# SerCharles/CN-RMA

Measured on AMD Instinct MI355X. Metric: scenes/sec fwd (40-view->192^3 voxel): dense unprojection + RMA + voxelise + FCAF3D + decode, higher is better.
Workload: dtype f32 (sparse conv f16x3: 22-bit operands, fp32 accumulate; value_f32_conv = exact fp32); 1 GPU; NS: 40 views x 256 ch x 480x640 fp32 maps (channels_last) -> grid 192x192x192, N=300, max_points=500000, FCAF3D MinkResNet34 + head, 1 HIP graph per scene, 3 in flight; M_rows=72216505, M_selected=500000, M_unique=496819

## Files before the change

### cn-rma_amd/csrc/rma.hip

```cpp
#include "common.h"

#include <stdlib.h>

namespace {

struct MarchParams {
  int V, H, W, X, Y, Z, N;
  float vs, ox, oy, oz, t_one, thr;
};

struct Ray {
  float ox, oy, oz, dx, dy, dz;
};

__device__ __forceinline__ Ray make_ray(const float* __restrict__ Pi, float u, float v) {
  float far_[3], o[3];
#pragma unroll
  for (int r = 0; r < 3; ++r) {
    float acc = Pi[r * 4 + 0] * u;
    acc = fmaf(Pi[r * 4 + 1], v, acc);
    acc = fmaf(Pi[r * 4 + 2], 1.0f, acc);
    acc = fmaf(Pi[r * 4 + 3], 1.0f, acc);
    far_[r] = acc;
    o[r] = Pi[r * 4 + 3];
// ... 722 lines not shown
  } else {
    if (tsdf == nullptr) return CNRMA_EINVAL;
    hipLaunchKernelGGL(neus_count_kernel, dim3((unsigned)ceil_div(R, 256)), dim3(256), 0, st, p, proj_inv, tsdf, count, wsum,
                       reinterpret_cast<int2*>(kept), cap, overflow);
  }
  CNRMA_LAUNCH_CHECK();
  return 0;
}

extern "C" int cnrma_rma_neus_march_f32(const float* proj_inv, const float* tsdf, const float* sig_table, int V, int H,
                                        int W, int X, int Y, int Z, float voxel_size, float ox, float oy, float oz,
                                        int n_steps, float t_one, float thr, int32_t* count, double* wsum, void* kept,
                                        int cap, int32_t* overflow, const void* skip_table, void* stream) {
  if (bad_dims(V, H, W, X, Y, Z, n_steps) || kept == nullptr || cap <= 0 || overflow == nullptr) return CNRMA_EINVAL;
  if (tsdf == nullptr && sig_table == nullptr) return CNRMA_EINVAL;
  MarchParams p = make_params(V, H, W, X, Y, Z, voxel_size, ox, oy, oz, n_steps, t_one, thr);
  return launch_march(p, proj_inv, tsdf, sig_table, count, wsum, kept, cap, overflow, nullptr, nullptr, 0, as_stream(stream),
                      sig_table ? reinterpret_cast<const uint8_t*>(skip_table) : nullptr);
}

extern "C" int cnrma_nchw_to_nhwc_march_f32(const float* feat_nchw, float* feat_nhwc, int C, const float* proj_inv,
                                            const float* tsdf, const float* sig_table, int V, int H, int W, int X, int Y,
                                            int Z, float voxel_size, float ox, float oy, float oz, int n_steps, float t_one,
                                            float thr, int32_t* count, double* wsum, void* kept, int cap, int32_t* overflow,
                                            const void* skip_table, void* stream) {
  if (bad_dims(V, H, W, X, Y, Z, n_steps) || kept == nullptr || cap <= 0 || overflow == nullptr || C <= 0 ||
      feat_nchw == nullptr || feat_nhwc == nullptr)
    return CNRMA_EINVAL;
  if (tsdf == nullptr && sig_table == nullptr) return CNRMA_EINVAL;
  MarchParams p = make_params(V, H, W, X, Y, Z, voxel_size, ox, oy, oz, n_steps, t_one, thr);
  return launch_march(p, proj_inv, tsdf, sig_table, count, wsum, kept, cap, overflow, feat_nchw, feat_nhwc, C, as_stream(stream),
                      sig_table ? reinterpret_cast<const uint8_t*>(skip_table) : nullptr);
}

template <int ELEM = 0, typename FT = float>
static int neus_emit_rows_any(const float* proj_inv, const FT* feat_nhwc, const FT* const* feat_ref, int V, int C, int H, int W,
                                            int n_steps, float t_one, const int32_t* row_offset, int64_t n_out,
                                            const int32_t* n_out_dev, const void* kept, int cap,
                                            const int32_t* sel_index, int64_t sel_cap, void* records,
                                            const float* w_div, float addx, float addy, float addz, float* out_xyz,
                                            int xyz_stride, float* out_w, int w_stride, float* out_feat,
                                            int feat_stride, int32_t* out_sample, void* stream) {
  if (V <= 0 || C <= 0 || H <= 0 || W <= 0 || n_out <= 0 || (kept != nullptr && cap <= 0) || records == nullptr ||
      (kept == nullptr && row_offset != nullptr) || (feat_nhwc == nullptr && feat_ref == nullptr && out_feat != nullptr))
    return CNRMA_EINVAL;
  MarchParams p = make_params(V, H, W, 1, 1, 1, 1.0f, 0.f, 0.f, 0.f, n_steps, t_one, 0.0f);
  EmitDst d{out_xyz, xyz_stride, out_w, w_stride, out_feat, feat_stride, out_sample, nullptr, w_div, addx, addy, addz};
  const int64_t R = (int64_t)V * H * W;
  hipStream_t st = as_stream(stream);
  int4* rec = reinterpret_cast<int4*>(records);
  if (kept != nullptr)
    hipLaunchKernelGGL(neus_scatter_records_kernel, dim3((unsigned)ceil_div(R, 256)), dim3(256), 0, st, R, row_offset,
                       reinterpret_cast<const int2*>(kept), cap, sel_index, sel_cap, n_out, rec);
  if (C % 256 == 0) {
    hipLaunchKernelGGL((neus_emit_rows_kernel<64, ELEM, FT>), dim3((unsigned)ceil_div(n_out * 64, 256)), dim3(256), 0, st, p, C,
                       proj_inv, feat_nhwc, feat_ref, n_out, n_out_dev, rec, d);
  } else if (C % 32 == 0) {
    hipLaunchKernelGGL((neus_emit_rows_kernel<8, ELEM, FT>), dim3((unsigned)ceil_div(n_out * 8, 256)), dim3(256), 0, st, p, C,
                       proj_inv, feat_nhwc, feat_ref, n_out, n_out_dev, rec, d);
  } else {
    hipLaunchKernelGGL((neus_emit_rows_kernel<2, ELEM, FT>), dim3((unsigned)ceil_div(n_out * 2, 256)), dim3(256), 0, st, p, C,
                       proj_inv, feat_nhwc, feat_ref, n_out, n_out_dev, rec, d);
  }
  CNRMA_LAUNCH_CHECK();
  return 0;
}

extern "C" int cnrma_rma_neus_emit_rows_f32(const float* proj_inv, const float* feat_nhwc, int V, int C, int H, int W,
                                            int n_steps, float t_one, const int32_t* row_offset, int64_t n_out,
                                            const int32_t* n_out_dev, const void* kept, int cap,
                                            const int32_t* sel_index, int64_t sel_cap, void* records,
                                            const float* w_div, float addx, float addy, float addz, float* out_xyz,
                                            int xyz_stride, float* out_w, int w_stride, float* out_feat,
                                            int feat_stride, int32_t* out_sample, void* stream) {
  return neus_emit_rows_any<0, float>(proj_inv, feat_nhwc, nullptr, V, C, H, W, n_steps, t_one, row_offset, n_out, n_out_dev, kept, cap,
                            sel_index, sel_cap, records, w_div, addx, addy, addz, out_xyz, xyz_stride, out_w, w_stride, out_feat,
                            feat_stride, out_sample, stream);
}

extern "C" int cnrma_rma_neus_emit_rows_ref_f32(const float* proj_inv, const float* const* feat_nhwc_ref, int V, int C, int H,
                                                int W, int n_steps, float t_one, const int32_t* row_offset, int64_t n_out,
                                                const int32_t* n_out_dev, const void* kept, int cap,
                                                const int32_t* sel_index, int64_t sel_cap, void* records,
                                                const float* w_div, float addx, float addy, float addz, float* out_xyz,
                                                int xyz_stride, float* out_w, int w_stride, float* out_feat,
                                                int feat_stride, int32_t* out_sample, void* stream) {
  if (feat_nhwc_ref == nullptr) return CNRMA_EINVAL;
  return neus_emit_rows_any<0, float>(proj_inv, nullptr, feat_nhwc_ref, V, C, H, W, n_steps, t_one, row_offset, n_out, n_out_dev, kept, cap,
                            sel_index, sel_cap, records, w_div, addx, addy, addz, out_xyz, xyz_stride, out_w, w_stride, out_feat,
                            feat_stride, out_sample, stream);
}

extern "C" int cnrma_rma_neus_emit_rows_h16(const float* proj_inv, const void* feat_nhwc, const void* const* feat_nhwc_ref, int elem,
                                            int V, int C, int H, int W, int n_steps, float t_one, const int32_t* row_offset,
                                            int64_t n_out, const int32_t* n_out_dev, const void* kept, int cap,
                                            const int32_t* sel_index, int64_t sel_cap, void* records, const float* w_div,
                                            float addx, float addy, float addz, float* out_xyz, int xyz_stride, float* out_w,
                                            int w_stride, float* out_feat, int feat_stride, int32_t* out_sample, void* stream) {
  if (!elem16_known(elem) || (feat_nhwc == nullptr) == (feat_nhwc_ref == nullptr) || C % 8 != 0 ||
      (reinterpret_cast<uintptr_t>(feat_nhwc) & 15) != 0)
    return CNRMA_EINVAL;
  const uint16_t* f = static_cast<const uint16_t*>(feat_nhwc);
  const uint16_t* const* fr = reinterpret_cast<const uint16_t* const*>(feat_nhwc_ref);
  if (elem == CNRMA_ELEM_F16)
    return neus_emit_rows_any<CNRMA_ELEM_F16, uint16_t>(proj_inv, f, fr, V, C, H, W, n_steps, t_one, row_offset, n_out, n_out_dev, kept,
                                                        cap, sel_index, sel_cap, records, w_div, addx, addy, addz, out_xyz, xyz_stride,
                                                        out_w, w_stride, out_feat, feat_stride, out_sample, stream);
// ... 139 lines not shown
```

### cn-rma_amd/csrc/sparse.hip

```cpp
#include <cstdio>
#include <type_traits>
#include "common.h"
#include "f16x3.h"

#include <hipcub/hipcub.hpp>

namespace {

struct UniqueWs {
  int32_t* slot;
  int32_t* idx;
  uint8_t* flag;
  void* scan;
  uint64_t* key_a; uint64_t* key_b;
  int32_t* val_a; int32_t* val_b;
  void* sort_tmp; size_t sort_tmp_bytes;
  int32_t* range_err;
};

size_t sort_temp_bytes(int64_t n) {
  size_t bytes = 0;
  hipError_t e = hipcub::DeviceRadixSort::SortPairs(nullptr, bytes, (const uint64_t*)nullptr, (uint64_t*)nullptr,
                                                    (const int32_t*)nullptr, (int32_t*)nullptr, (int)n, 0, 64, nullptr);
  if (e != hipSuccess || bytes == 0) bytes = (size_t)n * 16 + (1u << 20);
// ... 2121 lines not shown
#endif

__global__ __launch_bounds__(256) void convtr_coords_kernel(const int32_t* __restrict__ in_coords, int64_t n_cap,
                                                            const int32_t* __restrict__ n_dev, int half,
                                                            int32_t* __restrict__ out_coords) {
  const int64_t n = live_rows(n_cap, n_dev);
  const int64_t t = (int64_t)blockIdx.x * blockDim.x + threadIdx.x;
  if (t >= n * 8) return;
  const int m = (int)(t & 7);
  const int64_t i = t >> 3;
  int4 c = reinterpret_cast<const int4*>(in_coords)[i];
  c.y += ((m >> 2) & 1) * half;
  c.z += ((m >> 1) & 1) * half;
  c.w += (m & 1) * half;
  reinterpret_cast<int4*>(out_coords)[t] = c;
}

__global__ __launch_bounds__(256) void maxpool_kernel(const float* __restrict__ in, int C, const int32_t* __restrict__ nbr,
                                                      int K, float* __restrict__ out, int64_t no_cap,
                                                      const int32_t* __restrict__ no_dev) {
  const int64_t n = live_rows(no_cap, no_dev);
  const int64_t t = (int64_t)blockIdx.x * blockDim.x + threadIdx.x;
  if ((C & 3) == 0) {
    const int c4 = C >> 2;
    if (t >= n * c4) return;
    const int64_t o = t / c4;
    const int c = (int)(t - o * c4);
    float4 m = make_float4(-__builtin_inff(), -__builtin_inff(), -__builtin_inff(), -__builtin_inff());
    bool any = false;
    for (int k = 0; k < K; ++k) {
      const int32_t s = nbr[o * K + k];
      if (s >= 0) {
        const float4 v = reinterpret_cast<const float4*>(in)[(int64_t)s * c4 + c];
        m.x = fmaxf(m.x, v.x); m.y = fmaxf(m.y, v.y); m.z = fmaxf(m.z, v.z); m.w = fmaxf(m.w, v.w);
        any = true;
      }
    }
    reinterpret_cast<float4*>(out)[t] = any ? m : make_float4(0.f, 0.f, 0.f, 0.f);
    return;
  }
  if (t >= n * C) return;
  const int64_t o = t / C;
  const int c = (int)(t - o * C);
  float m = -__builtin_inff();
  bool any = false;
  for (int k = 0; k < K; ++k) {
    int32_t s = nbr[o * K + k];
    if (s >= 0) { m = fmaxf(m, in[(int64_t)s * C + c]); any = true; }
  }
  out[t] = any ? m : 0.0f;
}

struct StatsTerm {
  const float* __restrict__ in;
  __device__ __forceinline__ void operator()(int64_t i, double& a, double& b) const {
    const double v = (double)in[i];
    a = v;
    b = v * v;
  }
};

__device__ __forceinline__ void mask_grad(float& g, float yv, int act) {
  if (!(yv > 0.0f)) g = act == 2 ? g * (yv + 1.0f) : 0.0f;
}

struct GradTerm {
  const float* __restrict__ dy; const float* __restrict__ x; const float* __restrict__ y; int act;
  __device__ __forceinline__ void operator()(int64_t i, double& a, double& b) const {
    float gf = dy[i];
    if (y != nullptr) mask_grad(gf, y[i], act);
    const double g = (double)gf;
    a = g;
    b = g * (double)x[i];
  }
};

template <typename Term>
__global__ __launch_bounds__(256) void colsum_partial_kernel(Term term, int64_t n_cap, const int32_t* __restrict__ n_dev,
                                                             const int32_t* __restrict__ row0_dev, int C,
                                                             double* __restrict__ part) {
  const int64_t n = live_rows(n_cap, n_dev);
  const int64_t i0 = row0_dev != nullptr ? (int64_t)__builtin_nontemporal_load(row0_dev) * C : 0;
  const int c = threadIdx.x % C;
  const int groups = blockDim.x / C;
  const int gi = threadIdx.x / C;
  double s = 0.0, q = 0.0;
  if (gi < groups) {
    for (int64_t r = (int64_t)blockIdx.x * groups + gi; r < n; r += (int64_t)gridDim.x * groups) {
      double a, b;
      term(i0 + r * C + c, a, b);
      s += a;
      q += b;
    }
  }
  __shared__ double sm[2 * 256];
  sm[threadIdx.x] = s;
  sm[256 + threadIdx.x] = q;
  __syncthreads();
  if (threadIdx.x < C) {
    double ts = 0.0, tq = 0.0;
    for (int g = 0; g < groups; ++g) { ts += sm[g * C + threadIdx.x]; tq += sm[256 + g * C + threadIdx.x]; }
    part[(int64_t)blockIdx.x * 2 * C + threadIdx.x] = ts;
    part[(int64_t)blockIdx.x * 2 * C + C + threadIdx.x] = tq;
  }
}

__device__ __forceinline__ void colsum_channel(const double* __restrict__ part, int nblk, int C, int c, double& s_out, double& q_out) {
  __shared__ double ss[256], qq[256];
  double s = 0.0, q = 0.0;
  for (int b = threadIdx.x; b < nblk; b += 256) { s += part[(int64_t)b * 2 * C + c]; q += part[(int64_t)b * 2 * C + C + c]; }
  ss[threadIdx.x] = s; qq[threadIdx.x] = q;
  __syncthreads();
  for (int d = 128; d > 0; d >>= 1) {
    if ((int)threadIdx.x < d) { ss[threadIdx.x] += ss[threadIdx.x + d]; qq[threadIdx.x] += qq[threadIdx.x + d]; }
    __syncthreads();
  }
  if (threadIdx.x == 0) { s_out = ss[0]; q_out = qq[0]; }
}

__global__ __launch_bounds__(256) void colstats_final_kernel(const double* __restrict__ part, int nblk, int C, int64_t n_cap,
                                                             const int32_t* __restrict__ n_dev, double* __restrict__ stats,
                                                             float momentum, float* __restrict__ running_mean,
                                                             float* __restrict__ running_var, int64_t* __restrict__ batches) {
  const int c = blockIdx.x;
  double s = 0.0, q = 0.0;
  colsum_channel(part, nblk, C, c, s, q);
  if (threadIdx.x == 0) {
    const double nn = (double)live_rows(n_cap, n_dev);
    const double mean = s / nn;
    double var = q / nn - mean * mean;
    if (var < 0.0) var = 0.0;
    stats[c] = mean;
    stats[C + c] = var;
    if (running_mean != nullptr) running_mean[c] = (1.0f - momentum) * running_mean[c] + momentum * (float)mean;
    if (running_var != nullptr) running_var[c] = (1.0f - momentum) * running_var[c] + momentum * (float)(var * (nn / (nn - 1.0)));
    if (batches != nullptr && c == 0) *batches += 1;
  }
}

__global__ __launch_bounds__(256) void bn_backward_final_kernel(const double* __restrict__ part, int nblk, int C, int64_t n,
                                                                const double* __restrict__ stats, float eps,
                                                                float* __restrict__ dweight, float* __restrict__ dbias,
                                                                double* __restrict__ sums) {
  const int c = blockIdx.x;
  double s = 0.0, q = 0.0;
  colsum_channel(part, nblk, C, c, s, q);
  if (threadIdx.x == 0) {
    const double mean = stats[c], inv = 1.0 / sqrt(stats[C + c] + (double)eps);
    const double dg = (q - mean * s) * inv;
    if (dweight) dweight[c] = (float)dg;
// ... 15 lines not shown
  float v = (x - k.mean) * k.inv;
  if (weight) v = v * weight[c];
  if (bias) v = v + bias[c];
  return v;
}

__device__ __forceinline__ float norm_backward(float g, float x, NormCoef k, const float* weight,
                                               const double* sums, int C, int c) {
  const double* sums2 = sums + C;
  const float xhat = (x - k.mean) * k.inv;
  const float gain = weight ? weight[c] : 1.0f;
  return gain * k.inv * (g - (float)sums[c] - xhat * (float)sums2[c]);
}

__global__ __launch_bounds__(256) void instnorm_apply_kernel(const float* __restrict__ in, int64_t n_cap,
                                                             const int32_t* __restrict__ n_dev,
                                                             const int32_t* __restrict__ row0_dev, int C,
                                                             const double* __restrict__ stats,
                                                             const float* __restrict__ weight,
                                                             const float* __restrict__ bias, float eps, int relu,
                                                             float* __restrict__ out) {
  const int64_t n = live_rows(n_cap, n_dev);
  if (row0_dev != nullptr) {
    const int64_t r0 = (int64_t)__builtin_nontemporal_load(row0_dev) * C;
    in += r0;
    out += r0;
  }
  for (int64_t t = (int64_t)blockIdx.x * blockDim.x + threadIdx.x; t < n * C; t += (int64_t)gridDim.x * blockDim.x) {
    const int c = (int)(t % C);
    const float v = norm_forward(in[t], norm_coef(stats, C, c, eps), weight, bias, c);
    out[t] = relu ? fmaxf(v, 0.0f) : v;
  }
}

__global__ __launch_bounds__(256) void instnorm_maxpool_kernel(const float* __restrict__ in, int C,
                                                               const double* __restrict__ stats,
                                                               const float* __restrict__ weight,
                                                               const float* __restrict__ bias, float eps, int relu,
                                                               const int32_t* __restrict__ nbr, int K, float* __restrict__ out,
                                                               int64_t no_cap, const int32_t* __restrict__ no_dev,
                                                               float* __restrict__ out_amax) {
  const int64_t n = live_rows(no_cap, no_dev);
  const int64_t t = (int64_t)blockIdx.x * blockDim.x + threadIdx.x;
  const int c4 = C >> 2;
  float mx = 0.0f;
  if (t < n * c4) {
    const int64_t o = t / c4;
    const int c = (int)(t - o * c4) * 4;
    NormCoef kc[4];
#pragma unroll
    for (int j = 0; j < 4; ++j) kc[j] = norm_coef(stats, C, c + j, eps);
    float m[4] = {-__builtin_inff(), -__builtin_inff(), -__builtin_inff(), -__builtin_inff()};
    bool any = false;
    for (int k = 0; k < K; ++k) {
      const int32_t s_ = nbr[o * K + k];
      if (s_ >= 0) {
        const float4 q = *reinterpret_cast<const float4*>(in + (int64_t)s_ * C + c);
        const float x[4] = {q.x, q.y, q.z, q.w};
#pragma unroll
        for (int j = 0; j < 4; ++j) {
          float v = norm_forward(x[j], kc[j], weight, bias, c + j);
          if (relu) v = fmaxf(v, 0.0f);
          m[j] = fmaxf(m[j], v);
        }
        any = true;
      }
    }
    float4 r = any ? make_float4(m[0], m[1], m[2], m[3]) : make_float4(0.f, 0.f, 0.f, 0.f);
    *reinterpret_cast<float4*>(out + o * C + c) = r;
    mx = fmaxf(fmaxf(fabsf(r.x), fabsf(r.y)), fmaxf(fabsf(r.z), fabsf(r.w)));
  }
  if (out_amax != nullptr) {
    __shared__ float sh4[4];
    block_amax_publish(out_amax, mx, sh4);
  }
}

__global__ __launch_bounds__(256) void bn_apply_kernel(const float* __restrict__ in, int64_t n, int C, const double* __restrict__ stats,
                                                       const float* __restrict__ weight, const float* __restrict__ bias, float eps,
                                                       const float* __restrict__ residual, int relu, float* __restrict__ out) {
  const int64_t total4 = n * C / 4;
  for (int64_t t = (int64_t)blockIdx.x * blockDim.x + threadIdx.x; t < total4; t += (int64_t)gridDim.x * blockDim.x) {
    const int c = (int)((t * 4) % C);
    const float4 x = reinterpret_cast<const float4*>(in)[t];
    float4 r = make_float4(0.f, 0.f, 0.f, 0.f);
    if (residual) r = reinterpret_cast<const float4*>(residual)[t];
    const float xv[4] = {x.x, x.y, x.z, x.w}, rv[4] = {r.x, r.y, r.z, r.w};
    float o[4];
#pragma unroll
    for (int j = 0; j < 4; ++j) {
      float v = norm_forward(xv[j], norm_coef(stats, C, c + j, eps), weight, bias, c + j);
      if (residual) v = v + rv[j];
      o[j] = relu == 1 ? fmaxf(v, 0.0f) : (relu == 2 ? (v > 0.0f ? v : expm1f(v)) : v);
    }
    reinterpret_cast<float4*>(out)[t] = make_float4(o[0], o[1], o[2], o[3]);
  }
}

__global__ __launch_bounds__(256) void bn_backward_apply_kernel(const float* __restrict__ dy, const float* __restrict__ x,
                                                                int64_t n, int C, const double* __restrict__ stats,
                                                                const double* __restrict__ sums,
                                                                const float* __restrict__ weight, float eps,
                                                                float* __restrict__ dx) {
  for (int64_t t = (int64_t)blockIdx.x * blockDim.x + threadIdx.x; t < n * C; t += (int64_t)gridDim.x * blockDim.x) {
    const int c = (int)(t % C);
    dx[t] = norm_backward(dy[t], x[t], norm_coef(stats, C, c, eps), weight, sums, C, c);
  }
}

__global__ __launch_bounds__(256) void bn_backward_apply2_kernel(const float* __restrict__ dy, const float* __restrict__ x,
                                                                 const float* __restrict__ y, int act, int64_t n, int C,
                                                                 const double* __restrict__ stats, const double* __restrict__ sums,
                                                                 const float* __restrict__ weight, float eps,
                                                                 float* __restrict__ dx, float* __restrict__ dres) {
  const int64_t total4 = n * C / 4;
  for (int64_t t = (int64_t)blockIdx.x * blockDim.x + threadIdx.x; t < total4; t += (int64_t)gridDim.x * blockDim.x) {
    const int c = (int)((t * 4) % C);
    const float4 g4 = reinterpret_cast<const float4*>(dy)[t], x4 = reinterpret_cast<const float4*>(x)[t];
// ... 1190 lines not shown
      b += (hdr[k] + 127) & ~127;
    }
    base[K] = b;
    for (int k = 0; k <= K; ++k) hdr[64 + k] = base[k];
    hdr[64 + 33] = (int64_t)b <= pair_cap ? b : (int)pair_cap;
  }
  __syncthreads();
  for (int k = 0; k < K; ++k) {
    const int lo = base[k], hi = base[k + 1], live = lo + hdr[k];
    for (int t = lo / 128 + threadIdx.x; t < hi / 128 && (int64_t)t < pair_cap / 128; t += 256) tile_tap[t] = k;
    for (int r = live + threadIdx.x; r < hi && (int64_t)r < pair_cap; r += 256) pair_src[r] = -1;
  }
}

__global__ __launch_bounds__(256) void pairs_fill_kernel(const int32_t* __restrict__ nbr, int64_t no_cap,
                                                         const int32_t* __restrict__ no_dev, int K, int32_t* __restrict__ hdr,
                                                         int32_t* __restrict__ pair_src, int32_t* __restrict__ pos,
                                                         int64_t pair_cap) {
  __shared__ int hist[32], gbase[32];
  if (threadIdx.x < 32) hist[threadIdx.x] = 0;
  __syncthreads();
  const unsigned total = (unsigned)(live_rows(no_cap, no_dev) * K);
  const unsigned base = blockIdx.x * (256u * PAIR_EPT);
  int32_t src[PAIR_EPT];
#pragma unroll
  for (int j = 0; j < PAIR_EPT; ++j) {
    const unsigned t = base + j * 256u + threadIdx.x;
    src[j] = t < total ? nbr[t] : -1;
    if (src[j] >= 0) atomicAdd(&hist[tap_of(t, K)], 1);
  }
  __syncthreads();
  if (threadIdx.x < K) {
    const int c = hist[threadIdx.x];
    gbase[threadIdx.x] = c ? hdr[64 + threadIdx.x] + atomicAdd(&hdr[32 + threadIdx.x], c) : 0;
    hist[threadIdx.x] = 0;
  }
  __syncthreads();
#pragma unroll
  for (int j = 0; j < PAIR_EPT; ++j) {
    const unsigned t = base + j * 256u + threadIdx.x;
    if (t < total) {
      int32_t slot = -1;
      if (src[j] >= 0) {
        const int k = tap_of(t, K);
        slot = gbase[k] + atomicAdd(&hist[k], 1);
        if ((int64_t)slot < pair_cap) pair_src[slot] = src[j];
        else { slot = -1; hdr[64 + 34] = 1; }
      }
      pos[t] = slot;
    }
  }
}

template <int KT>
__global__ __launch_bounds__(256) void pairs_reduce_kernel(ConvArgs p, const int32_t* __restrict__ pos,
                                                           const float* __restrict__ prod) {
  const int64_t n_live = live_rows(p.no_cap, p.no_dev);
  const int C4 = p.Cout >> 2;
  const int64_t total = n_live * C4;
  const int K = KT > 0 ? KT : p.K;
  float mx = 0.0f;
  for (int64_t t = (int64_t)blockIdx.x * blockDim.x + threadIdx.x; t < total; t += (int64_t)gridDim.x * blockDim.x) {
    const int64_t o = t / C4;
    const int col = (int)(t % C4) * 4;
    float4 s = make_float4(0.f, 0.f, 0.f, 0.f);
    const int32_t* po = pos + o * K;
    if constexpr (KT > 0) {
      int32_t r[KT];
#pragma unroll
      for (int k = 0; k < KT; ++k) r[k] = po[k];
#pragma unroll
      for (int k = 0; k < KT; ++k)
        if (r[k] >= 0) {
          const float4 q = *reinterpret_cast<const float4*>(prod + (int64_t)r[k] * p.Cout + col);
          s.x += q.x; s.y += q.y; s.z += q.z; s.w += q.w;
        }
    } else {
      for (int k = 0; k < K; ++k) {
        const int32_t r = po[k];
        if (r >= 0) {
          const float4 q = *reinterpret_cast<const float4*>(prod + (int64_t)r * p.Cout + col);
          s.x += q.x; s.y += q.y; s.z += q.z; s.w += q.w;
        }
      }
    }
    float v[4] = {s.x, s.y, s.z, s.w};
#pragma unroll
    for (int j = 0; j < 4; ++j) {
      float x = v[j];
      if (p.scale) x = x * p.scale[col + j];
      if (p.shift) x = x + p.shift[col + j];
      if (p.residual) x = x + p.residual[o * p.Cout + col + j];
      v[j] = apply_act(x, p.act);
      mx = fmaxf(mx, fabsf(v[j]));
    }
    *reinterpret_cast<float4*>(p.out + o * p.Cout + col) = make_float4(v[0], v[1], v[2], v[3]);
  }
  if (p.out_amax != nullptr) {
    __shared__ float sh4[4];
    block_amax_publish(p.out_amax, mx, sh4);
  }
}

static size_t align256(size_t b) { return (b + 255) & ~(size_t)255; }

extern "C" size_t cnrma_sparse_conv_pairs_workspace_bytes(int64_t no_cap, int K, int Cout, int64_t pair_cap) {
  if (no_cap <= 0 || K <= 0 || Cout <= 0 || pair_cap <= 0) return 0;
  return align256(PAIR_HDR * 4) + align256((size_t)(pair_cap / 128 + 1) * 4) + align256((size_t)pair_cap * 4) +
         align256((size_t)no_cap * K * 4) + align256((size_t)pair_cap * Cout * 4);
}

static int launch_pairs(const float* in_feats, const float* in_amax, int Cin, const int32_t* nbr, const float* weight,
                        const void* image, const ConvArgs& epi, int64_t pair_cap, void* workspace, size_t workspace_bytes,
                        hipStream_t st) {
  const int K = epi.K, Cout = epi.Cout;
  const int64_t no_cap = epi.no_cap;
  if (workspace == nullptr || workspace_bytes < cnrma_sparse_conv_pairs_workspace_bytes(no_cap, K, Cout, pair_cap))
    return CNRMA_EINVAL;
  char* w = reinterpret_cast<char*>(workspace);
  int32_t* hdr = reinterpret_cast<int32_t*>(w);        w += align256(PAIR_HDR * 4);
  int32_t* tile_tap = reinterpret_cast<int32_t*>(w);   w += align256((size_t)(pair_cap / 128 + 1) * 4);
  int32_t* pair_src = reinterpret_cast<int32_t*>(w);   w += align256((size_t)pair_cap * 4);
  int32_t* pos = reinterpret_cast<int32_t*>(w);        w += align256((size_t)no_cap * K * 4);
  float* prod = reinterpret_cast<float*>(w);
  const hipError_t fe = cnrma_fill_bytes(hdr, 0, PAIR_HDR * 4, st);
  if (fe != hipSuccess) return -(int)fe;
  if (no_cap * K >= 0x7fffffffLL) return CNRMA_EINVAL;
  const int64_t blocks = ceil_div(no_cap * K, 256 * PAIR_EPT);
  hipLaunchKernelGGL(pairs_count_kernel, dim3((unsigned)blocks), dim3(256), 0, st, nbr, no_cap, epi.no_dev, K, hdr);
// ... 522 lines not shown
```

### cn-rma_amd/csrc/util.hip

```cpp
#include "common.h"

extern "C" int cnrma_abi_version(void) { return CNRMA_ABI_VERSION; }

extern "C" int cnrma_fill_bytes_u8(void* dst, int byte, size_t n_bytes, void* stream) {
  if (dst == nullptr || (n_bytes & 3) != 0 || (reinterpret_cast<uintptr_t>(dst) & 3) != 0) return CNRMA_EINVAL;
  if (n_bytes == 0) return 0;
  const hipError_t e = cnrma_fill_bytes(dst, byte, n_bytes, reinterpret_cast<hipStream_t>(stream));
  return e == hipSuccess ? 0 : -(int)e;
}

__global__ __launch_bounds__(256) void range_violations_kernel(const int32_t* __restrict__ v, const int32_t* __restrict__ lo,
                                                               const int32_t* __restrict__ hi, int n, int32_t* __restrict__ out) {
  __shared__ int sm[4];
  int c = 0;
  for (int i = threadIdx.x; i < n; i += 256) c += (v[i] < lo[i] || v[i] > hi[i]) ? 1 : 0;
  for (int o = 32; o > 0; o >>= 1) c += __shfl_down(c, o, 64);
  if ((threadIdx.x & 63) == 0) sm[threadIdx.x >> 6] = c;
  __syncthreads();
  if (threadIdx.x == 0) out[0] = sm[0] + sm[1] + sm[2] + sm[3];
}

extern "C" int cnrma_range_violations_i32(const int32_t* values, const int32_t* lo, const int32_t* hi, int n, int32_t* out,
                                          void* stream) {
  if (values == nullptr || lo == nullptr || hi == nullptr || out == nullptr || n <= 0 || n > 4096) return CNRMA_EINVAL;
// ... 260 lines not shown
  const int64_t view = blockIdx.z;
  const int64_t p0 = (int64_t)blockIdx.x * 64;
  const int c0 = blockIdx.y * 32;
  const uint16_t* s = src + view * C * HW;
  uint16_t* d = dst + view * C * HW;
  const int tx = threadIdx.x & 63, ty = threadIdx.x >> 6;
#pragma unroll
  for (int j = 0; j < 8; ++j) {
    int c = c0 + ty + 4 * j;
    int64_t p = p0 + tx;
    tile[ty + 4 * j][tx] = (c < C && p < HW) ? s[(int64_t)c * HW + p] : (uint16_t)0;
  }
  __syncthreads();
  const int cx = threadIdx.x & 31, py = threadIdx.x >> 5;
#pragma unroll
  for (int j = 0; j < 8; ++j) {
    int c = c0 + cx;
    int64_t p = p0 + py + 8 * j;
    if (c < C && p < HW) d[p * C + c] = tile[cx][py + 8 * j];
  }
}

__global__ __launch_bounds__(256) void nchw_to_nhwc_b16_v8_kernel(const uint16_t* __restrict__ src, uint16_t* __restrict__ dst, int C,
                                                                  int64_t HW) {
  __shared__ uint16_t tile[64][66];
  const int64_t view = blockIdx.z;
  const int64_t p0 = (int64_t)blockIdx.x * 64;
  const int c0 = blockIdx.y * 64;
  const uint16_t* s = src + view * C * HW;
  uint16_t* d = dst + view * C * HW;
  const int q = threadIdx.x & 7, r = threadIdx.x >> 3;
#pragma unroll
  for (int j = 0; j < 2; ++j) {
    const int c = r + 32 * j;
    uint4 v = make_uint4(0u, 0u, 0u, 0u);
    if (c0 + c < C && p0 + 8 * q < HW) v = *reinterpret_cast<const uint4*>(s + (int64_t)(c0 + c) * HW + p0 + 8 * q);
    const uint32_t w[4] = {v.x, v.y, v.z, v.w};
#pragma unroll
    for (int i = 0; i < 4; ++i) { tile[c][8 * q + 2 * i] = (uint16_t)(w[i] & 0xffffu); tile[c][8 * q + 2 * i + 1] = (uint16_t)(w[i] >> 16); }
  }
  __syncthreads();
#pragma unroll
  for (int j = 0; j < 2; ++j) {
    const int p = r + 32 * j;
    if (c0 + 8 * q < C && p0 + p < HW) {
      uint32_t w[4];
#pragma unroll
      for (int i = 0; i < 4; ++i) w[i] = (uint32_t)tile[8 * q + 2 * i][p] | ((uint32_t)tile[8 * q + 2 * i + 1][p] << 16);
      *reinterpret_cast<uint4*>(d + (p0 + p) * C + c0 + 8 * q) = make_uint4(w[0], w[1], w[2], w[3]);
    }
  }
}

__device__ __forceinline__ uint32_t row_hash(uint32_t seed, uint32_t i) {
  uint32_t x = i * 0x9E3779B1u + seed;
  x ^= x >> 16; x *= 0x7FEB352Du; x ^= x >> 15; x *= 0x846CA68Bu; x ^= x >> 16;
  return x;
}

__device__ __forceinline__ uint32_t select_key(const float* __restrict__ scores, uint32_t seed, uint32_t i) {
  if (scores == nullptr) return row_hash(seed, i);
  const uint32_t u = __float_as_uint(scores[i]);
  const uint32_t ordered = (u & 0x80000000u) ? ~u : (u | 0x80000000u);
  return ~ordered;
}

struct SampleWs {
  int32_t hist[3][2048];
  int32_t prefix[3];
  int32_t need[4];
  int32_t tie_count, pad;
  int32_t tie_idx[256];
  int32_t prefix2[3];
  int32_t pad3;
  int32_t list_count, pad2;
  uint64_t list[1024];
};
constexpr size_t SAMPLE_WS_ZEROED = offsetof(SampleWs, list);

__device__ __forceinline__ int key_digit(uint32_t k, int pass) {
  return pass == 0 ? (int)(k >> 21) : (pass == 1 ? (int)((k >> 10) & 2047u) : (int)(k & 1023u));
}
__device__ __forceinline__ bool key_matches(uint32_t k, int pass, const int32_t* prefix) {
  if (pass >= 1 && (int)(k >> 21) != prefix[0]) return false;
  if (pass >= 2 && (int)((k >> 10) & 2047u) != prefix[1]) return false;
  return true;
}

__device__ __forceinline__ void resolve_digit(const int32_t* __restrict__ hist, int need, int* digit, int* need_next,
                                              int* smem ) {
  int bins[8], local = 0;
#pragma unroll
  for (int j = 0; j < 8; ++j) { bins[j] = hist[8 * threadIdx.x + j]; local += bins[j]; }
  int* out = smem + 256 / 64 + 1;
  if (threadIdx.x == 0) { out[0] = 0; out[1] = 0; }
  int total;
  int ex = block_excl_scan<256>(local, smem, &total);
  if (ex < need && ex + local >= need) {
#pragma unroll
    for (int j = 0; j < 8; ++j) {
      if (ex < need && ex + bins[j] >= need) { out[0] = 8 * threadIdx.x + j; out[1] = need - ex; }
      ex += bins[j];
    }
  }
  __syncthreads();
  *digit = out[0];
  *need_next = out[1];
  __syncthreads();
}

// ... 5 lines not shown
  return seed_dev ? seed + 0x9E3779B9u * seed_dev[0] : seed;
}

__global__ __launch_bounds__(256) void sample_hist_kernel(const int32_t* __restrict__ m_dev, int64_t m_cap,
                                                          const float* __restrict__ scores, uint32_t seed,
                                                          const uint32_t* __restrict__ seed_dev, int pass, int n_keep,
                                                          SampleWs* __restrict__ ws) {
  seed = select_seed(seed, seed_dev);
  __shared__ int h[2048];
  __shared__ int rs[256 / 64 + 1 + 2];
  int32_t prefix[3] = {0, 0, 0};
  int need = n_keep;
  for (int q = 0; q < pass; ++q) {
    int nn;
    resolve_digit(ws->hist[q], need, &prefix[q], &nn, rs);
    need = nn;
  }
  for (int i = threadIdx.x; i < 2048; i += 256) h[i] = 0;
  __syncthreads();
  const int64_t M = select_rows(m_dev, m_cap);
  for (int64_t i = (int64_t)blockIdx.x * blockDim.x + threadIdx.x; i < M; i += (int64_t)gridDim.x * blockDim.x) {
    const uint32_t k = select_key(scores, seed, (uint32_t)i);
    if (key_matches(k, pass, prefix)) atomicAdd(&h[key_digit(k, pass)], 1);
  }
  __syncthreads();
  for (int i = threadIdx.x; i < 2048; i += 256)
    if (h[i]) atomicAdd(&ws->hist[pass][i], h[i]);
}

__global__ __launch_bounds__(256) void sample_ties_kernel(const int32_t* __restrict__ m_dev, int64_t m_cap,
                                                          const float* __restrict__ scores, uint32_t seed,
                                                          const uint32_t* __restrict__ seed_dev, int n_keep,
                                                          SampleWs* __restrict__ ws) {
  seed = select_seed(seed, seed_dev);
  __shared__ int rs[256 / 64 + 1 + 2];
  int32_t prefix[3];
  int need = n_keep;
  for (int q = 0; q < 3; ++q) {
    int nn;
    resolve_digit(ws->hist[q], need, &prefix[q], &nn, rs);
    need = nn;
  }
  if (blockIdx.x == 0 && threadIdx.x == 0) {
    ws->prefix[0] = prefix[0]; ws->prefix[1] = prefix[1]; ws->prefix[2] = prefix[2];
    ws->need[0] = n_keep; ws->need[3] = need;
  }
  const int64_t M = select_rows(m_dev, m_cap);
  const uint32_t key = ((uint32_t)prefix[0] << 21) | ((uint32_t)prefix[1] << 10) | (uint32_t)prefix[2];
  for (int64_t i = (int64_t)blockIdx.x * blockDim.x + threadIdx.x; i < M; i += (int64_t)gridDim.x * blockDim.x) {
    if (select_key(scores, seed, (uint32_t)i) == key) {
      const int slot = atomicAdd(&ws->tie_count, 1);
      if (slot < 256) ws->tie_idx[slot] = (int32_t)i;
    }
  }
}

__global__ __launch_bounds__(1024) void sample_tie_select_kernel(const int32_t* __restrict__ m_dev, int64_t m_cap,
                                                                const float* __restrict__ scores, uint32_t seed,
                                                                const uint32_t* __restrict__ seed_dev,
                                                                SampleWs* __restrict__ ws) {
  if (ws->tie_count <= 256) return;
  seed = select_seed(seed, seed_dev);
  __shared__ int h[2048];
  __shared__ int sh_digit, sh_need;
  const int64_t M = select_rows(m_dev, m_cap);
  const uint32_t key = ((uint32_t)ws->prefix[0] << 21) | ((uint32_t)ws->prefix[1] << 10) | (uint32_t)ws->prefix[2];
  int32_t prefix2[3] = {0, 0, 0};
  int need = ws->need[3];
  for (int pass = 0; pass < 3; ++pass) {
    for (int i = threadIdx.x; i < 2048; i += 1024) h[i] = 0;
    __syncthreads();
    for (int64_t i = threadIdx.x; i < M; i += 1024) {
      if (select_key(scores, seed, (uint32_t)i) != key) continue;
      const uint32_t k2 = (uint32_t)i;
      if (key_matches(k2, pass, prefix2)) atomicAdd(&h[key_digit(k2, pass)], 1);
    }
    __syncthreads();
    if (threadIdx.x == 0) {
      int cum = 0, d = 0, nn = 0;
      for (int bin = 0; bin < 2048; ++bin) {
        if (cum < need && cum + h[bin] >= need) { d = bin; nn = need - cum; break; }
        cum += h[bin];
      }
      sh_digit = d; sh_need = nn;
    }
    __syncthreads();
    prefix2[pass] = sh_digit;
    need = sh_need;
    __syncthreads();
  }
  if (threadIdx.x == 0) { ws->prefix2[0] = prefix2[0]; ws->prefix2[1] = prefix2[1]; ws->prefix2[2] = prefix2[2]; }
}

__device__ __forceinline__ int32_t select_tie_bound(const SampleWs* __restrict__ ws, int32_t* sh_bound, int* rs) {
  (void)rs;
  if (threadIdx.x == 0) {
    const int cnt = min(ws->tie_count, 256), need = ws->need[3];
    int32_t bound = -1;
    if (ws->tie_count > 256) {
      bound = (int32_t)(((uint32_t)ws->prefix2[0] << 21) | ((uint32_t)ws->prefix2[1] << 10) | (uint32_t)ws->prefix2[2]);
    } else {
      for (int r = 0; r < need; ++r) {
        int32_t best = 0x7FFFFFFF;
        for (int q = 0; q < cnt; ++q) { const int32_t v = ws->tie_idx[q]; if (v > bound && v < best) best = v; }
        bound = best;
      }
// ... 80 lines not shown
  if (m1 > M) m1 = M;
  int c = 0;
  for (int64_t i = m0; i < m1; ++i) {
    const uint32_t k = row_hash(seed, (uint32_t)i);
    c += (all || k < key || (k == key && (int32_t)i <= tie_bound)) ? 1 : 0;
  }
  counts[r] = c;
}

__global__ __launch_bounds__(256) void select_scatter_records_kernel(int64_t R, const int32_t* __restrict__ off,
                                                                     const int32_t* __restrict__ sel_off,
                                                                     const int2* __restrict__ kept, int cap,
                                                                     const int32_t* __restrict__ m_dev, int64_t m_cap,
                                                                     uint32_t seed, const uint32_t* __restrict__ seed_dev,
                                                                     const SampleWs* __restrict__ ws, int n_keep,
                                                                     int64_t rec_cap, int4* __restrict__ rec) {
  seed = select_seed(seed, seed_dev);
  const int64_t M = select_rows(m_dev, m_cap);
  __shared__ int32_t sh_bound;
  __shared__ int rs[256 / 64 + 1 + 2];
  const int32_t tie_bound = select_tie_bound(ws, &sh_bound, rs);
  const bool all = M <= n_keep;
  const uint32_t key = ((uint32_t)ws->prefix[0] << 21) | ((uint32_t)ws->prefix[1] << 10) | (uint32_t)ws->prefix[2];
  const int64_t r = (int64_t)blockIdx.x * blockDim.x + threadIdx.x;
  if (r >= R) return;
  const int64_t m0 = off[r];
  int64_t m1 = off[r + 1];
  if (m1 > M) m1 = M;
  int64_t j = sel_off[r];
  for (int64_t i = m0; i < m1; ++i) {
    const uint32_t k = row_hash(seed, (uint32_t)i);
    if (all || k < key || (k == key && (int32_t)i <= tie_bound)) {
      if (j < rec_cap && i - m0 < cap) {
        const int2 kv = kept[r * cap + (i - m0)];
        rec[j] = make_int4((int)r, kv.y, kv.x, 0);
      }
      ++j;
    }
  }
}

}

extern "C" size_t cnrma_sample_workspace_bytes(void) { return sizeof(SampleWs); }

static int run_select(const int32_t* m_dev, const float* scores, int64_t m_cap, int n_keep, uint32_t seed,
                      const uint32_t* seed_dev, uint8_t* mask, void* workspace, hipStream_t st, int64_t* out_idx = nullptr) {
  if (m_cap <= 0 || n_keep <= 0 || m_cap >= ((int64_t)1 << 31)) return CNRMA_EINVAL;
  SampleWs* ws = reinterpret_cast<SampleWs*>(workspace);
  hipError_t e = cnrma_fill_bytes(ws, 0, SAMPLE_WS_ZEROED, st);
  if (e != hipSuccess) return -(int)e;
  int blocks = (int)(m_cap / 2048 + 1);
  if (blocks > 1024) blocks = 1024;
  for (int pass = 0; pass < 3; ++pass)
    hipLaunchKernelGGL(sample_hist_kernel, dim3(blocks), dim3(256), 0, st, m_dev, m_cap, scores, seed, seed_dev, pass,
                       n_keep, ws);
  hipLaunchKernelGGL(sample_ties_kernel, dim3(blocks), dim3(256), 0, st, m_dev, m_cap, scores, seed, seed_dev, n_keep, ws);
  hipLaunchKernelGGL(sample_tie_select_kernel, dim3(1), dim3(1024), 0, st, m_dev, m_cap, scores, seed, seed_dev, ws);
  if (mask != nullptr) {
    hipLaunchKernelGGL(sample_mask_kernel, dim3(blocks), dim3(256), 0, st, m_dev, m_cap, scores, seed, seed_dev, ws, n_keep,
                       mask);
  } else if (out_idx == nullptr) {
  } else {
    hipLaunchKernelGGL(sample_collect_kernel, dim3(blocks), dim3(256), 0, st, m_dev, m_cap, scores, ws, n_keep);
    hipLaunchKernelGGL(topk_sort_kernel, dim3(1), dim3(1024), 0, st, ws, n_keep, out_idx);
  }
  CNRMA_LAUNCH_CHECK();
  return 0;
}

extern "C" int cnrma_sample_mask(const int32_t* m_dev, int64_t m_cap, int n_keep, uint32_t seed, const uint32_t* seed_dev,
                                 uint8_t* mask, void* workspace, void* stream) {
  if (m_dev == nullptr) return CNRMA_EINVAL;
  return run_select(m_dev, nullptr, m_cap, n_keep, seed, seed_dev, mask, workspace, as_stream(stream));
}

extern "C" int cnrma_topk_mask_f32(const float* scores, const int32_t* n_dev, int64_t n_cap, int k, uint8_t* mask,
                                   void* workspace, void* stream) {
  if (scores == nullptr || n_dev == nullptr) return CNRMA_EINVAL;
  return run_select(n_dev, scores, n_cap, k, 0u, nullptr, mask, workspace, as_stream(stream));
}

extern "C" int cnrma_rma_select_records(const int32_t* row_offset, int64_t R, const void* kept, int cap, const int32_t* m_dev,
                                        int64_t m_cap, int n_keep, uint32_t seed, const uint32_t* seed_dev, void* sample_ws,
                                        int32_t* ray_counts, int32_t* ray_offsets, void* scan_ws, int64_t rec_cap,
                                        void* records, int32_t* n_sel, void* stream) {
  if (row_offset == nullptr || kept == nullptr || m_dev == nullptr || R <= 0 || cap <= 0 || records == nullptr ||
      ray_counts == nullptr || ray_offsets == nullptr || n_sel == nullptr)
    return CNRMA_EINVAL;
  hipStream_t st = as_stream(stream);
  int rc = run_select(m_dev, nullptr, m_cap, n_keep, seed, seed_dev, nullptr, sample_ws, st, nullptr);
  if (rc != 0) return rc;
  const SampleWs* ws = reinterpret_cast<const SampleWs*>(sample_ws);
  const unsigned blocks = (unsigned)ceil_div(R, 256);
  hipLaunchKernelGGL(select_count_segments_kernel, dim3(blocks), dim3(256), 0, st, R, row_offset, m_dev, m_cap, seed, seed_dev,
                     ws, n_keep, ray_counts);
  rc = run_scan<int32_t, 0>(ray_counts, ray_offsets, n_sel, R, scan_ws, st);
  if (rc != 0) return rc;
  hipLaunchKernelGGL(select_scatter_records_kernel, dim3(blocks), dim3(256), 0, st, R, row_offset, ray_offsets,
                     reinterpret_cast<const int2*>(kept), cap, m_dev, m_cap, seed, seed_dev, ws, n_keep, rec_cap,
                     reinterpret_cast<int4*>(records));
  CNRMA_LAUNCH_CHECK();
  return 0;
}

extern "C" int cnrma_topk_indices_f32(const float* scores, const int32_t* n_dev, int64_t n_cap, int k, int64_t* out_idx,
                                      void* workspace, void* stream) {
  if (scores == nullptr || n_dev == nullptr || out_idx == nullptr || k > 1024) return CNRMA_EINVAL;
  return run_select(n_dev, scores, n_cap, k, 0u, nullptr, nullptr, workspace, as_stream(stream), out_idx);
}

// ... 60 lines not shown
```

Baseline: 65.23 scenes/s.

## Invert row hash for sampling passes and vectorise colsum, pooling and pair reduce

```diff
diff --git a/cn-rma_amd/csrc/rma.hip b/cn-rma_amd/csrc/rma.hip
--- a/cn-rma_amd/csrc/rma.hip
+++ b/cn-rma_amd/csrc/rma.hip
@@ -798,7 +798,10 @@
   if (kept != nullptr)
     hipLaunchKernelGGL(neus_scatter_records_kernel, dim3((unsigned)ceil_div(R, 256)), dim3(256), 0, st, R, row_offset,
                        reinterpret_cast<const int2*>(kept), cap, sel_index, sel_cap, n_out, rec);
-  if (C % 256 == 0) {
+  if (out_feat == nullptr) {
+    hipLaunchKernelGGL((neus_emit_rows_kernel<1, ELEM, FT>), dim3((unsigned)ceil_div(n_out, 256)), dim3(256), 0, st, p, C,
+                       proj_inv, feat_nhwc, feat_ref, n_out, n_out_dev, rec, d);
+  } else if (C % 256 == 0) {
     hipLaunchKernelGGL((neus_emit_rows_kernel<64, ELEM, FT>), dim3((unsigned)ceil_div(n_out * 64, 256)), dim3(256), 0, st, p, C,
                        proj_inv, feat_nhwc, feat_ref, n_out, n_out_dev, rec, d);
   } else if (C % 32 == 0) {
diff --git a/cn-rma_amd/csrc/sparse.hip b/cn-rma_amd/csrc/sparse.hip
--- a/cn-rma_amd/csrc/sparse.hip
+++ b/cn-rma_amd/csrc/sparse.hip
@@ -2197,6 +2197,7 @@
 }
 
 struct StatsTerm {
+  static constexpr bool QUADS = true;
   const float* __restrict__ in;
   __device__ __forceinline__ void operator()(int64_t i, double& a, double& b) const {
     const double v = (double)in[i];
@@ -2210,6 +2211,7 @@
 }
 
 struct GradTerm {
+  static constexpr bool QUADS = false;
   const float* __restrict__ dy; const float* __restrict__ x; const float* __restrict__ y; int act;
   __device__ __forceinline__ void operator()(int64_t i, double& a, double& b) const {
     float gf = dy[i];
@@ -2219,6 +2221,40 @@
     b = g * (double)x[i];
   }
 };
+
+constexpr int COLSUM_ROWS = 8;
+
+__device__ __forceinline__ void colsum_rows_quads(const float* __restrict__ in, int64_t n, int C, int groups, double* sm) {
+  const int c4 = C >> 2;
+  if ((int)threadIdx.x >= groups * c4) return;
+  const int gi = threadIdx.x / c4, c = (threadIdx.x % c4) * 4;
+  const float* __restrict__ col = in + c;
+  const int64_t step = (int64_t)gridDim.x * groups;
+  double s[4] = {0.0, 0.0, 0.0, 0.0}, q[4] = {0.0, 0.0, 0.0, 0.0};
+  auto add = [&](const float4& x) {
+    const float xs[4] = {x.x, x.y, x.z, x.w};
+#pragma unroll
+    for (int j = 0; j < 4; ++j) {
+      const double v = (double)xs[j];
+      s[j] += v;
+      q[j] += v * v;
+    }
+  };
+  int64_t r = (int64_t)blockIdx.x * groups + gi;
+  for (; r + (COLSUM_ROWS - 1) * step < n; r += COLSUM_ROWS * step) {
+    float4 x[COLSUM_ROWS];
+#pragma unroll
+    for (int u = 0; u < COLSUM_ROWS; ++u) x[u] = *reinterpret_cast<const float4*>(col + (r + u * step) * C);
+#pragma unroll
+    for (int u = 0; u < COLSUM_ROWS; ++u) add(x[u]);
+  }
+  for (; r < n; r += step) add(*reinterpret_cast<const float4*>(col + r * C));
+#pragma unroll
+  for (int j = 0; j < 4; ++j) {
+    sm[gi * C + c + j] = s[j];
+    sm[256 + gi * C + c + j] = q[j];
+  }
+}
 
 template <typename Term>
 __global__ __launch_bounds__(256) void colsum_partial_kernel(Term term, int64_t n_cap, const int32_t* __restrict__ n_dev,
@@ -2229,18 +2265,25 @@
   const int c = threadIdx.x % C;
   const int groups = blockDim.x / C;
   const int gi = threadIdx.x / C;
-  double s = 0.0, q = 0.0;
-  if (gi < groups) {
-    for (int64_t r = (int64_t)blockIdx.x * groups + gi; r < n; r += (int64_t)gridDim.x * groups) {
-      double a, b;
-      term(i0 + r * C + c, a, b);
-      s += a;
-      q += b;
-    }
-  }
   __shared__ double sm[2 * 256];
-  sm[threadIdx.x] = s;
-  sm[256 + threadIdx.x] = q;
+  bool quads = false;
+  if constexpr (Term::QUADS) {
+    quads = (C & 3) == 0 && (reinterpret_cast<uintptr_t>(term.in) & 15) == 0;
+    if (quads) colsum_rows_quads(term.in + i0, n, C, groups, sm);
+  }
+  if (!quads) {
+    double s = 0.0, q = 0.0;
+    if (gi < groups) {
+      for (int64_t r = (int64_t)blockIdx.x * groups + gi; r < n; r += (int64_t)gridDim.x * groups) {
+        double a, b;
+        term(i0 + r * C + c, a, b);
+        s += a;
+        q += b;
+      }
+    }
+    sm[threadIdx.x] = s;
+    sm[256 + threadIdx.x] = q;
+  }
   __syncthreads();
   if (threadIdx.x < C) {
     double ts = 0.0, tq = 0.0;
@@ -2362,18 +2405,31 @@
     for (int j = 0; j < 4; ++j) kc[j] = norm_coef(stats, C, c + j, eps);
     float m[4] = {-__builtin_inff(), -__builtin_inff(), -__builtin_inff(), -__builtin_inff()};
     bool any = false;
-    for (int k = 0; k < K; ++k) {
-      const int32_t s_ = nbr[o * K + k];
-      if (s_ >= 0) {
-        const float4 q = *reinterpret_cast<const float4*>(in + (int64_t)s_ * C + c);
-        const float x[4] = {q.x, q.y, q.z, q.w};
-#pragma unroll
-        for (int j = 0; j < 4; ++j) {
-          float v = norm_forward(x[j], kc[j], weight, bias, c + j);
-          if (relu) v = fmaxf(v, 0.0f);
-          m[j] = fmaxf(m[j], v);
-        }
-        any = true;
+    auto take = [&](const float4& q) {
+      const float x[4] = {q.x, q.y, q.z, q.w};
+#pragma unroll
+      for (int j = 0; j < 4; ++j) {
+        float v = norm_forward(x[j], kc[j], weight, bias, c + j);
+        if (relu) v = fmaxf(v, 0.0f);
+        m[j] = fmaxf(m[j], v);
+      }
+      any = true;
+    };
+    if (K <= 8) {
+      int32_t s_[8];
+#pragma unroll
+      for (int k = 0; k < 8; ++k) s_[k] = k < K ? nbr[o * K + k] : -1;
+      float4 q[8];
+#pragma unroll
+      for (int k = 0; k < 8; ++k)
+        q[k] = s_[k] >= 0 ? *reinterpret_cast<const float4*>(in + (int64_t)s_[k] * C + c) : make_float4(0.f, 0.f, 0.f, 0.f);
+#pragma unroll
+      for (int k = 0; k < 8; ++k)
+        if (s_[k] >= 0) take(q[k]);
+    } else {
+      for (int k = 0; k < K; ++k) {
+        const int32_t s_ = nbr[o * K + k];
+        if (s_ >= 0) take(*reinterpret_cast<const float4*>(in + (int64_t)s_ * C + c));
       }
     }
     float4 r = any ? make_float4(m[0], m[1], m[2], m[3]) : make_float4(0.f, 0.f, 0.f, 0.f);
@@ -3670,6 +3726,48 @@
   }
 }
 
+__device__ __forceinline__ float4 pairs_sum27_wave(const int32_t* __restrict__ pos, const float* __restrict__ prod, int Cout,
+                                                   int64_t o0, int rows, int row_in_wave, int64_t n_live, int col) {
+  const int lane = threadIdx.x & 63;
+  const int64_t e0 = o0 * 27, e_end = n_live * 27;
+  const int32_t v0 = (lane < rows * 27 && e0 + lane < e_end) ? pos[e0 + lane] : -1;
+  const int32_t v1 = (64 + lane < rows * 27 && e0 + 64 + lane < e_end) ? pos[e0 + 64 + lane] : -1;
+  const uint64_t b0 = __ballot(v0 >= 0), b1 = __ballot(v1 >= 0);
+  const int sh = row_in_wave * 27;
+  uint64_t bits;
+  if (sh == 0) bits = b0;
+  else if (sh < 64) bits = (b0 >> sh) | (b1 << (64 - sh));
+  else bits = b1 >> (sh - 64);
+  uint32_t m = (uint32_t)bits & ((1u << 27) - 1);
+  auto next = [&]() -> int32_t {
+    const int e = sh + (m ? __builtin_ctz(m) : 0);
+    const int32_t a = __shfl(v0, e & 63), b = __shfl(v1, e & 63);
+    const int32_t r = m ? (e < 64 ? a : b) : -1;
+    m &= m - 1;
+    return r;
+  };
+  float4 s = make_float4(0.f, 0.f, 0.f, 0.f);
+  constexpr int FIRST = 4;
+  int32_t r[FIRST];
+#pragma unroll
+  for (int i = 0; i < FIRST; ++i) r[i] = next();
+  float4 q[FIRST];
+#pragma unroll
+  for (int i = 0; i < FIRST; ++i)
+    q[i] = r[i] >= 0 ? *reinterpret_cast<const float4*>(prod + (int64_t)r[i] * Cout + col) : make_float4(0.f, 0.f, 0.f, 0.f);
+#pragma unroll
+  for (int i = 0; i < FIRST; ++i)
+    if (r[i] >= 0) { s.x += q[i].x; s.y += q[i].y; s.z += q[i].z; s.w += q[i].w; }
+  while (__any(m != 0)) {
+    const int32_t rr = next();
+    if (rr >= 0) {
+      const float4 qq = *reinterpret_cast<const float4*>(prod + (int64_t)rr * Cout + col);
+      s.x += qq.x; s.y += qq.y; s.z += qq.z; s.w += qq.w;
+    }
+  }
+  return s;
+}
+
 template <int KT>
 __global__ __launch_bounds__(256) void pairs_reduce_kernel(ConvArgs p, const int32_t* __restrict__ pos,
                                                            const float* __restrict__ prod) {
@@ -3677,22 +3775,30 @@
   const int C4 = p.Cout >> 2;
   const int64_t total = n_live * C4;
   const int K = KT > 0 ? KT : p.K;
+  const int lane = threadIdx.x & 63;
+  const bool by_wave = KT == 27 && (C4 == 16 || C4 == 32 || C4 == 64);
   float mx = 0.0f;
-  for (int64_t t = (int64_t)blockIdx.x * blockDim.x + threadIdx.x; t < total; t += (int64_t)gridDim.x * blockDim.x) {
+  for (int64_t base = (int64_t)blockIdx.x * blockDim.x + (threadIdx.x - lane); base < total;
+       base += (int64_t)gridDim.x * blockDim.x) {
+    const int64_t t = base + lane;
     const int64_t o = t / C4;
     const int col = (int)(t % C4) * 4;
     float4 s = make_float4(0.f, 0.f, 0.f, 0.f);
+    if (by_wave) s = pairs_sum27_wave(pos, prod, p.Cout, base / C4, 64 / C4, lane / C4, n_live, col);
+    if (t >= total) continue;
     const int32_t* po = pos + o * K;
     if constexpr (KT > 0) {
-      int32_t r[KT];
-#pragma unroll
-      for (int k = 0; k < KT; ++k) r[k] = po[k];
-#pragma unroll
-      for (int k = 0; k < KT; ++k)
-        if (r[k] >= 0) {
-          const float4 q = *reinterpret_cast<const float4*>(prod + (int64_t)r[k] * p.Cout + col);
-          s.x += q.x; s.y += q.y; s.z += q.z; s.w += q.w;
-        }
+      if (!by_wave) {
+        int32_t r[KT];
+#pragma unroll
+        for (int k = 0; k < KT; ++k) r[k] = po[k];
+#pragma unroll
+        for (int k = 0; k < KT; ++k)
+          if (r[k] >= 0) {
+            const float4 q = *reinterpret_cast<const float4*>(prod + (int64_t)r[k] * p.Cout + col);
+            s.x += q.x; s.y += q.y; s.z += q.z; s.w += q.w;
+          }
+      }
     } else {
       for (int k = 0; k < K; ++k) {
         const int32_t r = po[k];
diff --git a/cn-rma_amd/csrc/util.hip b/cn-rma_amd/csrc/util.hip
--- a/cn-rma_amd/csrc/util.hip
+++ b/cn-rma_amd/csrc/util.hip
@@ -336,10 +336,24 @@
   }
 }
 
+constexpr uint32_t HASH_MUL_I = 0x9E3779B1u, HASH_MUL_1 = 0x7FEB352Du, HASH_MUL_2 = 0x846CA68Bu;
 __device__ __forceinline__ uint32_t row_hash(uint32_t seed, uint32_t i) {
-  uint32_t x = i * 0x9E3779B1u + seed;
-  x ^= x >> 16; x *= 0x7FEB352Du; x ^= x >> 15; x *= 0x846CA68Bu; x ^= x >> 16;
+  uint32_t x = i * HASH_MUL_I + seed;
+  x ^= x >> 16; x *= HASH_MUL_1; x ^= x >> 15; x *= HASH_MUL_2; x ^= x >> 16;
   return x;
+}
+
+constexpr uint32_t mul_inverse(uint32_t a) {
+  uint32_t x = a;
+  for (int i = 0; i < 5; ++i) x *= 2u - a * x;
+  return x;
+}
+constexpr uint32_t HASH_INV_I = mul_inverse(HASH_MUL_I), HASH_INV_1 = mul_inverse(HASH_MUL_1), HASH_INV_2 = mul_inverse(HASH_MUL_2);
+static_assert(HASH_MUL_I * HASH_INV_I == 1u && HASH_MUL_1 * HASH_INV_1 == 1u && HASH_MUL_2 * HASH_INV_2 == 1u, "mul_inverse");
+__device__ __forceinline__ uint32_t row_unhash(uint32_t seed, uint32_t k) {
+  uint32_t x = k;
+  x ^= x >> 16; x *= HASH_INV_2; x ^= (x >> 15) ^ (x >> 30); x *= HASH_INV_1; x ^= x >> 16;
+  return (x - seed) * HASH_INV_I;
 }
 
 __device__ __forceinline__ uint32_t select_key(const float* __restrict__ scores, uint32_t seed, uint32_t i) {
@@ -451,6 +465,54 @@
       const int slot = atomicAdd(&ws->tie_count, 1);
       if (slot < 256) ws->tie_idx[slot] = (int32_t)i;
     }
+  }
+}
+
+__global__ __launch_bounds__(256) void sample_hist_inverse_kernel(const int32_t* __restrict__ m_dev, int64_t m_cap, uint32_t seed,
+                                                                  const uint32_t* __restrict__ seed_dev, int pass, int n_keep,
+                                                                  SampleWs* __restrict__ ws) {
+  seed = select_seed(seed, seed_dev);
+  __shared__ int h[2048];
+  __shared__ int rs[256 / 64 + 1 + 2];
+  int32_t prefix[3] = {0, 0, 0};
+  int need = n_keep;
+  for (int q = 0; q < pass; ++q) {
+    int nn;
+    resolve_digit(ws->hist[q], need, &prefix[q], &nn, rs);
+    need = nn;
+  }
+  for (int i = threadIdx.x; i < 2048; i += 256) h[i] = 0;
+  __syncthreads();
+  const int64_t M = select_rows(m_dev, m_cap);
+  const uint32_t head = ((uint32_t)prefix[0] << 21) | ((uint32_t)prefix[1] << 10);
+  const uint32_t tails = pass == 1 ? 1u << 21 : 1u << 10;
+  for (uint32_t j = blockIdx.x * blockDim.x + threadIdx.x; j < tails; j += gridDim.x * blockDim.x) {
+    const uint32_t k = head | j;
+    if ((int64_t)row_unhash(seed, k) < M) atomicAdd(&h[key_digit(k, pass)], 1);
+  }
+  __syncthreads();
+  for (int i = threadIdx.x; i < 2048; i += 256)
+    if (h[i]) atomicAdd(&ws->hist[pass][i], h[i]);
+}
+
+__global__ __launch_bounds__(256) void sample_tie_inverse_kernel(const int32_t* __restrict__ m_dev, int64_t m_cap, uint32_t seed,
+                                                                 const uint32_t* __restrict__ seed_dev, int n_keep,
+                                                                 SampleWs* __restrict__ ws) {
+  seed = select_seed(seed, seed_dev);
+  __shared__ int rs[256 / 64 + 1 + 2];
+  int32_t prefix[3];
+  int need = n_keep;
+  for (int q = 0; q < 3; ++q) {
+    int nn;
+    resolve_digit(ws->hist[q], need, &prefix[q], &nn, rs);
+    need = nn;
+  }
+  if (threadIdx.x == 0) {
+    ws->prefix[0] = prefix[0]; ws->prefix[1] = prefix[1]; ws->prefix[2] = prefix[2];
+    ws->need[0] = n_keep; ws->need[3] = need;
+    const uint32_t key = ((uint32_t)prefix[0] << 21) | ((uint32_t)prefix[1] << 10) | (uint32_t)prefix[2];
+    const uint32_t i = row_unhash(seed, key);
+    if ((int64_t)i < select_rows(m_dev, m_cap)) { ws->tie_count = 1; ws->tie_idx[0] = (int32_t)i; }
   }
 }
 
@@ -637,11 +699,18 @@
   if (e != hipSuccess) return -(int)e;
   int blocks = (int)(m_cap / 2048 + 1);
   if (blocks > 1024) blocks = 1024;
-  for (int pass = 0; pass < 3; ++pass)
-    hipLaunchKernelGGL(sample_hist_kernel, dim3(blocks), dim3(256), 0, st, m_dev, m_cap, scores, seed, seed_dev, pass,
-                       n_keep, ws);
-  hipLaunchKernelGGL(sample_ties_kernel, dim3(blocks), dim3(256), 0, st, m_dev, m_cap, scores, seed, seed_dev, n_keep, ws);
-  hipLaunchKernelGGL(sample_tie_select_kernel, dim3(1), dim3(1024), 0, st, m_dev, m_cap, scores, seed, seed_dev, ws);
+  if (scores == nullptr) {
+    hipLaunchKernelGGL(sample_hist_kernel, dim3(blocks), dim3(256), 0, st, m_dev, m_cap, scores, seed, seed_dev, 0, n_keep, ws);
+    hipLaunchKernelGGL(sample_hist_inverse_kernel, dim3(256), dim3(256), 0, st, m_dev, m_cap, seed, seed_dev, 1, n_keep, ws);
+    hipLaunchKernelGGL(sample_hist_inverse_kernel, dim3(1), dim3(256), 0, st, m_dev, m_cap, seed, seed_dev, 2, n_keep, ws);
+    hipLaunchKernelGGL(sample_tie_inverse_kernel, dim3(1), dim3(256), 0, st, m_dev, m_cap, seed, seed_dev, n_keep, ws);
+  } else {
+    for (int pass = 0; pass < 3; ++pass)
+      hipLaunchKernelGGL(sample_hist_kernel, dim3(blocks), dim3(256), 0, st, m_dev, m_cap, scores, seed, seed_dev, pass,
+                         n_keep, ws);
+    hipLaunchKernelGGL(sample_ties_kernel, dim3(blocks), dim3(256), 0, st, m_dev, m_cap, scores, seed, seed_dev, n_keep, ws);
+    hipLaunchKernelGGL(sample_tie_select_kernel, dim3(1), dim3(1024), 0, st, m_dev, m_cap, scores, seed, seed_dev, ws);
+  }
   if (mask != nullptr) {
     hipLaunchKernelGGL(sample_mask_kernel, dim3(blocks), dim3(256), 0, st, m_dev, m_cap, scores, seed, seed_dev, ws, n_keep,
                        mask);
```

Result: no change. 65.01 scenes/s (-0.3%).
